# yekaizhou/duet

Measured on AMD Instinct MI355X. Metric: SV support-read marks clustered+phased /sec; bit-exact phased_sv.vcf vs ref, higher is better.
Workload: dtype u32/u64 integer + f64 threshold compares; 1 GPU; BASELINE configs[1]: synthetic 1 contig, 1001116 SV marks / 100000 candidates / 159991 tagged reads, resident in HBM; step = ef_classify + ef_finalize_own, two launches (phasing, E/F; ef_seed_sort 0: ; marks_per_gpu=1001116, candidates_per_gpu=100000, reads_per_gpu=159991, parallelism=contig-sharded x1, svlen_thres=50, suppread_thres=2, device_preheat_steps=2500

## Files before the change

### duet_amd/csrc/duet_ef.hip

```cpp

#include <hip/hip_runtime.h>
#include <hip/hip_ext.h>
#include <stdint.h>
#include <stdio.h>
#include <stdlib.h>
#include <string.h>
#include <string>
#include <vector>

#include "duet_ef.h"
#include "duet_internal.h"

#pragma clang fp contract(off)

namespace {

#ifdef DUET_STAMPS
#define STAMP(k, i) do { if (threadIdx.x == 0 && p.stamps) p.stamps[((size_t)(k) * 65536 + blockIdx.x) * 8 + (i)] = wall_clock64(); } while (0)
#else
#define STAMP(k, i) do { } while (0)
#endif

#include "duet_seeds.hip.h"

constexpr uint32_t kPcMax = DUET_PC_MAX;

constexpr uint8_t kNeedNearest = 4;
constexpr uint8_t kClass2 = 8;
constexpr uint8_t kClass2Slow = 16;
constexpr uint8_t kDivZero = 32;

constexpr int kCandPerBlock = 256;
constexpr int kChunk = 3072;
constexpr int kStageIt = kChunk / (kCandPerBlock * 4);
constexpr int kSmallK = 64;
constexpr int kSortThreads = 1024;
constexpr uint32_t kSortLds = 15360;
constexpr uint32_t kLongCnt = 16;
constexpr uint32_t kLongTiles = 256;
constexpr uint32_t kMaxRuns = 32;
constexpr uint32_t kSeedTab = 4096;
constexpr uint32_t kFewRuns = 4;
constexpr uint32_t kOneLds = 4096;
constexpr uint32_t kC2Quota = 64;
constexpr int kC2Groups = 2;
constexpr int kC2Words = 2 + 6 * kC2Groups;

struct Vote {
    uint32_t hap1, hap2, hap0, allhap;
    uint64_t t1, t2;
};

__device__ int decide(int cls, const Vote &v, uint32_t deg, uint32_t svread, uint32_t refread)
{
    const bool hp_le = deg != 0 && 4ull * v.allhap <= 3ull * deg, hp_gt = deg != 0 && !hp_le;
    const double a1 = v.hap1 > 0 ? (double)v.t1 / (double)v.hap1 : 0.0;
    const double a2 = v.hap2 > 0 ? (double)v.t2 / (double)v.hap2 : 0.0;
    const double sv_ratio = (double)svread / (double)((uint64_t)svread + (uint64_t)refread);
    const uint64_t lo = v.t1 < v.t2 ? v.t1 : v.t2;
    const uint64_t hi = v.t1 < v.t2 ? v.t2 : v.t1;
    const double totsc_ratio = lo > 0 ? (double)hi / (double)lo : 0.0;
    const uint64_t onehap = lo == 0 ? hi : 0;
    const double diff = fabs(a2 - a1);
    int pred = 0;
    if (cls == 0) {
        if (sv_ratio == 1.0 && svread >= 4) pred = 3;
    } else if (cls == 2) {
        if (sv_ratio >= 0.72) {
            if (diff <= 1369.50) { if (svread >= 3) pred = 3; }
            else { if (v.hap0 >= 6) pred = 3; }
        }
    } else {
        const bool gate = (hp_le && diff <= 2400.0) || hp_gt;
        if (onehap != 0) {
            if (sv_ratio <= 0.24) pred = 0;
            else if (sv_ratio <= 0.9) { if (gate) pred = a1 > 0 ? 1 : 2; }
            else { if (gate) pred = 3; }
        } else {
            if (sv_ratio <= 0.3) pred = 0;
            else if (sv_ratio <= 0.45) pred = refread > 10 ? 0 : (v.t1 > v.t2 ? 1 : 2);
            else if (sv_ratio <= 0.75) pred = totsc_ratio <= 9.72 ? 3 : (v.t1 > v.t2 ? 1 : 2);
            else pred = 3;
        }
    }
    return pred;
}

__device__ __forceinline__ int decide01_int(int cls, const Vote &v, uint32_t deg, uint32_t svread, uint32_t refread, bool &need_fp)
{
    const uint64_t sr64 = (uint64_t)svread + (uint64_t)refread;
    const uint32_t sr = (uint32_t)sr64, s = svread;
    const uint32_t t1 = (uint32_t)v.t1, t2 = (uint32_t)v.t2, h1 = v.hap1, h2 = v.hap2;
    need_fp = (sr64 >> 26) != 0 || ((v.t1 | v.t2) >> 21) != 0 || ((h1 | h2) >> 8) != 0 || (deg >> 28) != 0;
    if (cls == 0) return (refread == 0 && svread >= 4) ? 3 : 0;
    const uint32_t s4 = s << 2, s10 = (s << 3) + (s << 1), s20 = s10 << 1, s25 = (s << 4) + (s << 3) + s;
    const uint32_t sr3 = (sr << 1) + sr, sr6 = sr3 << 1, sr9 = (sr << 3) + sr;
    const bool le024 = s25 <= sr6, le09 = s10 <= sr9, le03 = s10 <= sr3, le045 = s20 <= sr9, le075 = s4 <= sr3;
    const bool hp_le = deg != 0 && (v.allhap << 2) <= (deg << 1) + deg, hp_gt = deg != 0 && !hp_le;
    const uint32_t lo = t1 < t2 ? t1 : t2, hi = t1 < t2 ? t2 : t1;
    bool diff_le = true;
    if (h1 != 0 && h2 != 0) {
        const int32_t N = (int32_t)__umul24(t2, h1) - (int32_t)__umul24(t1, h2);
        const uint32_t A = (uint32_t)(N < 0 ? -N : N), B = __umul24(__umul24(h1, h2), 2400u);
        need_fp = need_fp || (A == B && t1 != 0 && t2 != 0);
        diff_le = A <= B;
    } else if ((h1 | h2) != 0) {
        diff_le = (h1 != 0 ? t1 : t2) <= __umul24(h1 | h2, 2400u);
    }
    const bool gate = (hp_le && diff_le) || hp_gt;
    int pred = 0;
    if (lo == 0 && hi != 0) {
        if (le024) pred = 0;
        else if (le09) { if (gate) pred = (h1 != 0 && t1 != 0) ? 1 : 2; }
        else { if (gate) pred = 3; }
    } else {
        const bool ratio_le = lo == 0 || __umul24(hi, 25u) <= __umul24(lo, 243u);
        if (le03) pred = 0;
        else if (le045) pred = refread > 10 ? 0 : (t1 > t2 ? 1 : 2);
        else if (le075) pred = ratio_le ? 3 : (t1 > t2 ? 1 : 2);
        else pred = 3;
    }
    return pred;
}

__device__ __forceinline__ uint32_t find_contig(const uint32_t *__restrict__ ctg_off, uint32_t K, uint32_t c)
{
    uint32_t lo = 0, hi = K;
    while (hi - lo > 1) {
        const uint32_t mid = (lo + hi) >> 1;
        if (ctg_off[mid] <= c) lo = mid; else hi = mid;
    }
    return lo;
}

struct Params {
    uint32_t K, C, M;
    uint32_t n_reads;
    const uint64_t *untagged;
    const uint64_t *read_tag;
    const uint32_t *cand_pos, *cand_svlen, *cand_svread, *cand_refread;
    const uint8_t *cand_gt_ok;
    const uint32_t *cand_off, *mark_read;
    uint32_t svlen_thres, suppread_thres;
    const uint32_t *ctg_off;
    const uint8_t *ctg_start;
    const uint32_t *blk_ctg;
    uint64_t *blk_rec;
    uint64_t *seed_ent;
    uint32_t *onebuf;
    uint32_t one_cap;
    uint32_t *tmpbuf;
    uint32_t *n_one;
    uint32_t *c2rec;
    uint32_t c2_fixed, c2_cap;
    uint32_t *status;
    uint8_t *out_pred;
    uint32_t *out_ps;
    uint32_t n_small;
    uint32_t ctg_small[kSmallK + 1];
    const uint32_t *dyn_c;
    const uint16_t *cand_contig;
    uint32_t dbg;
    uint32_t heavy_t;
    unsigned long long *stamps;
};


struct CandState {
    uint32_t first_ps = kEmpty;
    bool multi = false;
    uint32_t ps_a = kEmpty, ps_b = kEmpty, n_a = 0, n_b = 0, nv = 0;
    uint32_t a1 = 0, a2 = 0, b1 = 0, b2 = 0;
    uint32_t tb1 = 0, tb2 = 0;
    uint64_t TA1 = 0, TA2 = 0;
    bool more = false;

    __device__ __forceinline__ uint32_t n_ps() const { return first_ps == kEmpty ? 0u : (multi ? 2u : 1u); }
    __device__ __forceinline__ uint32_t seed() const { return ps_a; }
};

__device__ __forceinline__ uint32_t sel0(unsigned long long mask, uint32_t v)
{
    uint32_t d;
    asm("v_cndmask_b32_e64 %0, 0, %1, %2" : "=v"(d) : "v"(v), "s"(mask));
    return d;
}
__device__ __forceinline__ uint32_t selv(unsigned long long mask, uint32_t a, uint32_t b)
{
    uint32_t d;
    asm("v_cndmask_b32_e64 %0, %1, %2, %3" : "=v"(d) : "v"(a), "v"(b), "s"(mask));
    return d;
}
__device__ __forceinline__ uint32_t inc(uint32_t x, unsigned long long mask)
{
    uint32_t d;
    asm("v_addc_co_u32_e64 %0, vcc, 0, %1, %2" : "=v"(d) : "v"(x), "s"(mask) : "vcc");
    return d;
}

__device__ __forceinline__ void consume_range(CandState &st, const uint64_t *s_tag, uint32_t lo, uint32_t hi, uint32_t cs)
{
    uint32_t mn = st.first_ps;
    uint32_t mx = st.first_ps == kEmpty ? 0u : st.first_ps + 1u;
    uint32_t pa1 = 0, pa2 = 0, pb1 = 0, pb2 = 0;
    unsigned long long has_a = __ballot(st.ps_a != kEmpty), has_b = __ballot(st.ps_b != kEmpty), more = 0;
    uint32_t nv = 0, nb = 0, ps_a = st.ps_a, ps_b = st.ps_b;
    const uint64_t *q = s_tag + (lo < hi ? lo - cs : 0u), *qe = q + (lo < hi ? hi - lo : 0u);
    for (; q < qe; ++q) {
        const uint64_t tag = *q;
        const uint32_t ps = (uint32_t)tag, w = (uint32_t)(tag >> 32);
        const uint32_t pc = w & 0x3FFFFFFFu;
        const unsigned long long vm = __ballot(pc <= kPcMax);
        const unsigned long long m1 = __ballot((int32_t)w >= 0x40000000), m2 = __ballot((int32_t)w < -0x40000000);
        mn = min(mn, ps);
        mx = max(mx, ps + 1u);
        nv = inc(nv, vm);
        ps_a = selv(vm & ~has_a, ps_a, ps);
        has_a |= vm;
        const unsigned long long ina = vm & __ballot(ps == ps_a), rest = vm ^ ina;
        ps_b = selv(rest & ~has_b, ps_b, ps);
        has_b |= rest;
        const unsigned long long inb = rest & __ballot(ps == ps_b);
        more |= rest ^ inb;
        nb = inc(nb, inb);
        const uint32_t pcx = pc | (1u << 24);
        pa1 += sel0(ina & m1, pcx); pa2 += sel0(ina & m2, pcx);
        pb1 += sel0(inb & m1, pcx); pb2 += sel0(inb & m2, pcx);
    }
    const uint32_t lane = threadIdx.x & 63u;
    st.ps_a = ps_a; st.ps_b = ps_b;
    st.more = st.more || ((more >> lane) & 1ull) != 0ull;
    st.multi = st.multi || (mn != kEmpty && mn + 1u != mx);
    st.first_ps = mn;
    st.nv += nv; st.n_b += nb;
    st.n_a = st.more ? (st.ps_a != kEmpty ? 1u : 0u) : st.nv - st.n_b;
    st.a1 += pa1 >> 24; st.a2 += pa2 >> 24; st.b1 += pb1 >> 24; st.b2 += pb2 >> 24;
    st.TA1 += pa1 & 0xFFFFFFu; st.TA2 += pa2 & 0xFFFFFFu;
    st.tb1 += pb1 & 0xFFFFFFu; st.tb2 += pb2 & 0xFFFFFFu;
}

__device__ __forceinline__ uint32_t wave_sum(uint32_t v)
{
    v += (uint32_t)__builtin_amdgcn_update_dpp(0, (int)v, 0xB1, 0xF, 0xF, false);
    v += (uint32_t)__builtin_amdgcn_update_dpp(0, (int)v, 0x4E, 0xF, 0xF, false);
    v += (uint32_t)__builtin_amdgcn_update_dpp(0, (int)v, 0x124, 0xF, 0xF, false);
    v += (uint32_t)__builtin_amdgcn_update_dpp(0, (int)v, 0x128, 0xF, 0xF, false);
    v += (uint32_t)__builtin_amdgcn_update_dpp(0, (int)v, 0x142, 0xA, 0xF, false);
    v += (uint32_t)__builtin_amdgcn_update_dpp(0, (int)v, 0x143, 0xC, 0xF, false);
    return (uint32_t)__builtin_amdgcn_readlane((int)v, 63);
}

template <uint32_t J>
__device__ __forceinline__ uint32_t lane_xor(uint32_t v)
{
    if constexpr (J == 1) return (uint32_t)__builtin_amdgcn_update_dpp(0, (int)v, 0xB1, 0xF, 0xF, false);
    else if constexpr (J == 2) return (uint32_t)__builtin_amdgcn_update_dpp(0, (int)v, 0x4E, 0xF, 0xF, false);
    else if constexpr (J == 4) {
        const int r = __builtin_amdgcn_update_dpp((int)v, (int)v, 0x104, 0xF, 0x5, false);
        return (uint32_t)__builtin_amdgcn_update_dpp(r, (int)v, 0x114, 0xF, 0xA, false);
    } else if constexpr (J == 8) return (uint32_t)__builtin_amdgcn_update_dpp(0, (int)v, 0x128, 0xF, 0xF, false);
    else return (uint32_t)__shfl_xor((int)v, (int)J, 64);
}

template <uint32_t KK, uint32_t J>
__device__ __forceinline__ uint32_t bitonic_step(uint32_t v, uint32_t lane)
{
    const uint32_t o = lane_xor<J>(v);
    const bool up = KK == 64u || (lane & KK) == 0u, low = (lane & J) == 0u;
    v = (low == up) ? min(v, o) : max(v, o);
    if constexpr (J > 1) return bitonic_step<KK, J / 2>(v, lane);
    else return v;
}
__device__ __forceinline__ uint32_t wave_sort64(uint32_t v, uint32_t lane)
{
    v = bitonic_step<2, 1>(v, lane);
    v = bitonic_step<4, 2>(v, lane);
    v = bitonic_step<8, 4>(v, lane);
    v = bitonic_step<16, 8>(v, lane);
    v = bitonic_step<32, 16>(v, lane);
    return bitonic_step<64, 32>(v, lane);
}

__device__ __forceinline__ void consume_heavy(CandState &st, const uint64_t *s_tag, uint32_t lo, uint32_t hi, uint32_t cs, uint32_t lane,
                                              uint32_t h)
{
    uint32_t first_ps = (uint32_t)__builtin_amdgcn_readlane((int)st.first_ps, h);
    uint32_t ps_a = (uint32_t)__builtin_amdgcn_readlane((int)st.ps_a, h);
    uint32_t ps_b = (uint32_t)__builtin_amdgcn_readlane((int)st.ps_b, h);
    bool multi = false, more = false;
    uint32_t nv = 0, n_a = 0, n_b = 0, a1 = 0, a2 = 0, b1 = 0, b2 = 0;
    uint32_t ta1 = 0, ta2 = 0, tb1 = 0, tb2 = 0;
    for (uint32_t m0 = lo; m0 < hi; m0 += 64u) {
        const uint32_t m = m0 + lane;
        const uint64_t tag = m < hi ? s_tag[m - cs] : kUntagged;
        const uint32_t ps = (uint32_t)tag, w = (uint32_t)(tag >> 32);
        const uint32_t pc = w & 0x3FFFFFFFu, hap = w >> 30;
        const bool voter = pc <= kPcMax;
        const unsigned long long tmask = __ballot(ps != kEmpty);
        if (first_ps == kEmpty && tmask) first_ps = (uint32_t)__builtin_amdgcn_readlane((int)ps, (uint32_t)__ffsll((long long)tmask) - 1u);
        multi = multi || __ballot(ps != first_ps && ps != kEmpty) != 0ull;
        const unsigned long long vmask = __ballot(voter);
        if (ps_a == kEmpty && vmask) ps_a = (uint32_t)__builtin_amdgcn_readlane((int)ps, (uint32_t)__ffsll((long long)vmask) - 1u);
        const bool in_a = voter && ps == ps_a;
        const unsigned long long amask = __ballot(in_a);
        const unsigned long long rmask = vmask & ~amask;
        if (ps_b == kEmpty && rmask) ps_b = (uint32_t)__builtin_amdgcn_readlane((int)ps, (uint32_t)__ffsll((long long)rmask) - 1u);
        const bool in_b = voter && !in_a && ps == ps_b;
        const unsigned long long bmask = __ballot(in_b);
        more = more || (rmask & ~bmask) != 0ull;
        const bool is1 = hap == 1, is2 = hap == 2;
        const unsigned long long m1 = __ballot(is1), m2 = __ballot(is2);
        nv += (uint32_t)__popcll(vmask);
        n_a += (uint32_t)__popcll(amask); n_b += (uint32_t)__popcll(bmask);
        a1 += (uint32_t)__popcll(amask & m1); a2 += (uint32_t)__popcll(amask & m2);
        b1 += (uint32_t)__popcll(bmask & m1); b2 += (uint32_t)__popcll(bmask & m2);
        ta1 += (in_a && is1) ? pc : 0u; ta2 += (in_a && is2) ? pc : 0u;
        tb1 += (in_b && is1) ? pc : 0u; tb2 += (in_b && is2) ? pc : 0u;
    }
    const uint32_t s_a1 = a1 ? wave_sum(ta1) : 0u, s_a2 = a2 ? wave_sum(ta2) : 0u;
    const uint32_t s_b1 = b1 ? wave_sum(tb1) : 0u, s_b2 = b2 ? wave_sum(tb2) : 0u;
    if (lane == h) {
        st.first_ps = first_ps; st.multi = st.multi || multi;
        st.ps_a = ps_a; st.ps_b = ps_b; st.more = st.more || more;
        st.nv += nv; st.n_a += n_a; st.n_b += n_b;
        st.a1 += a1; st.a2 += a2; st.b1 += b1; st.b2 += b2;
        st.TA1 += s_a1; st.TA2 += s_a2; st.tb1 += s_b1; st.tb2 += s_b2;
    }
}

struct TileRecs {
    const ulonglong4 *p;
    __device__ __forceinline__ ulonglong4 operator[](uint32_t b) const { return p[2 * (size_t)b]; }
    __device__ __forceinline__ ulonglong4 second(uint32_t b) const { return p[2 * (size_t)b + 1]; }
};

struct TileShared {
    uint32_t seed[kCandPerBlock];
    uint32_t wcnt[kCandPerBlock / 64], wlast[kCandPerBlock / 64], wclean[kCandPerBlock / 64];
    uint32_t c2n;
    uint32_t c2base;
};

__device__ __forceinline__ void store_summary(const Params &p, uint32_t slot, const CandState &st)
{
    uint32_t *rec = p.c2rec + (size_t)slot * kC2Words;
    const uint32_t ng = (st.n_a != 0) + (st.n_b != 0);
    rec[0] = st.nv; rec[1] = ng;
    rec[2] = st.ps_a; rec[3] = st.n_a; rec[4] = st.a1; rec[5] = st.a2;
    rec[6] = (uint32_t)st.TA1; rec[7] = (uint32_t)st.TA2;
    rec[8] = st.ps_b; rec[9] = st.n_b; rec[10] = st.b1; rec[11] = st.b2; rec[12] = st.tb1; rec[13] = st.tb2;
}

__device__ __forceinline__ uint32_t decide_store(const Params &p, TileShared &sh, uint32_t tile, bool live, uint32_t c,
                                                 bool active, bool divzero, const CandState &st, uint32_t deg,
                                                 uint32_t svread, uint32_t refread, uint32_t &c2_rank)
{
    uint8_t code = 0;
    uint32_t ps_out = 0;
    bool want_seed = false;
    const uint32_t n_ps = st.n_ps();
    const bool c2 = active && n_ps == 2;
    const bool c2_fast = c2 && !st.more && deg < 500000u;
    const uint32_t rank = c2_fast ? atomicAdd(&sh.c2n, 1u) : kEmpty;
    c2_rank = rank;
    if (live) {
        want_seed = (active || divzero) && (n_ps == 1) && st.seed() != kEmpty;
        if (divzero) {
            code = kDivZero;
        } else if (active) {
            if (c2) {
                if (rank < kC2Quota) {
                    const uint32_t slot = tile * kC2Quota + rank;
                    store_summary(p, slot, st);
                    code = kClass2;
                    ps_out = slot;
                } else {
                    code = kClass2Slow;
                }
            } else {
                Vote v;
                v.hap1 = st.a1; v.hap2 = st.a2; v.hap0 = 0;
                v.allhap = st.a1 + st.a2;
                v.t1 = st.TA1; v.t2 = st.TA2;
                bool need_fp = false;
                int pred = (p.dbg & DUET_DBG_EF_FP_DECIDE) ? 0 : decide01_int((int)n_ps, v, deg, svread, refread, need_fp);
                need_fp = need_fp || (p.dbg & DUET_DBG_EF_FP_DECIDE) != 0;
                if (need_fp) pred = decide((int)n_ps, v, deg, svread, refread);
                code = (uint8_t)pred;
                ps_out = st.ps_a == kEmpty ? 0u : st.ps_a;
                if (n_ps == 0 || (st.a1 == 0 && st.a2 == 0)) code |= kNeedNearest;
            }
        }
        p.out_pred[c] = code;
        p.out_ps[c] = ps_out;
    }
    return want_seed ? st.seed() : kEmpty;
}

__device__ __forceinline__ void seeds_tile(const Params &p, TileShared &sh, uint32_t tile, uint32_t tid, uint32_t c,
                                           uint32_t is_start)
{
    const uint32_t seed = sh.seed[tid];
    const bool want_seed = seed != kEmpty;
    const uint32_t lane = tid & 63u, wave = tid >> 6;
    const unsigned long long wmask = __ballot(want_seed);
    const unsigned long long smask = __ballot(is_start != 0);
    const unsigned long long upto = lane == 63 ? ~0ull : ((1ull << (lane + 1)) - 1ull);
    if (lane == 0) {
        if (wmask) {
            const uint32_t li = 63u - (uint32_t)__clzll(wmask);
            sh.wlast[wave] = sh.seed[wave * 64 + li];
            sh.wclean[wave] = (li == 63 || (smask >> (li + 1)) == 0) ? 1u : 0u;
        } else {
            sh.wlast[wave] = kEmpty;
            sh.wclean[wave] = 0;
        }
    }
    __syncthreads();
    bool keep = want_seed;
    if (want_seed) {
        const unsigned long long lower = wmask & (upto >> 1);
        if (lower) {
            const uint32_t pl = 63u - (uint32_t)__clzll(lower);
            const unsigned long long between = smask & upto & ~((1ull << (pl + 1)) - 1ull);
            keep = !(between == 0 && sh.seed[wave * 64 + pl] == seed);
        } else if (wave > 0) {
            keep = !((smask & upto) == 0 && sh.wclean[wave - 1] && sh.wlast[wave - 1] == seed);
        }
    }
    const unsigned long long mask = __ballot(keep);
    if (lane == 0) sh.wcnt[wave] = (uint32_t)__popcll(mask);
    __syncthreads();
    uint32_t before = 0, total = 0;
#pragma unroll
    for (uint32_t w = 0; w < kCandPerBlock / 64; ++w) {
        before += w < wave ? sh.wcnt[w] : 0u;
        total += sh.wcnt[w];
    }
    if (keep) {
        const uint32_t at = before + (uint32_t)__popcll(mask & (upto >> 1));
        const uint64_t e = ((uint64_t)c << 32) | seed;
        if (at < 7) p.blk_rec[(size_t)tile * 8 + 1 + at] = e;
        if (at >= 3) p.seed_ent[(size_t)tile * kCandPerBlock + at] = e;
    }
    if (tid == 0) p.blk_rec[(size_t)tile * 8] = total;
}

__device__ __forceinline__ void stage_load_marks(const Params &p, uint4 (&r)[kStageIt], uint32_t cs, uint32_t m_end, uint32_t tid)
{
#pragma unroll
    for (int it = 0; it < kStageIt; ++it) {
        const uint32_t m = cs + 4u * (tid + it * kCandPerBlock);
        r[it] = *reinterpret_cast<const uint4 *>(p.mark_read + (m < m_end ? m : cs));
    }
}

__device__ __forceinline__ void stage_gather(const Params &p, uint64_t (&t)[4 * kStageIt], const uint4 (&r)[kStageIt])
{
#pragma unroll
    for (int it = 0; it < kStageIt; ++it) {
        const uint32_t idx[4] = {r[it].x, r[it].y, r[it].z, r[it].w};
#pragma unroll
        for (int j = 0; j < 4; ++j) {
            const uint64_t *a = idx[j] < p.n_reads ? p.read_tag + idx[j] : p.untagged;
            t[4 * it + j] = *a;
        }
    }
}

__device__ __forceinline__ void stage_store(uint64_t *s_tag, const uint64_t (&t)[4 * kStageIt], uint32_t cs, uint32_t m_end, uint32_t tid)
{
#pragma unroll
    for (int it = 0; it < kStageIt; ++it) {
        const uint32_t i = 4u * (tid + it * kCandPerBlock);
        if (cs + i < m_end) {
#pragma unroll
            for (int j = 0; j < 4; ++j) s_tag[i + j] = t[4 * it + j];
        }
    }
}

template <bool VEC, bool DYN = false>
__global__ __launch_bounds__(kCandPerBlock, 6) void ef_classify(const Params p)
{
    __shared__ uint64_t s_tag[kChunk];
    __shared__ uint32_t s_off[kCandPerBlock + 1];
    __shared__ TileShared sh;

    const uint32_t tid = threadIdx.x;
    STAMP(0, 0);
    const uint32_t n_cands = DYN ? *p.dyn_c : p.C;
    for (uint32_t tile = blockIdx.x; !DYN || tile * (uint32_t)kCandPerBlock < n_cands; tile += gridDim.x) {
        const uint32_t c0 = tile * kCandPerBlock;
        const uint32_t nc = min((uint32_t)kCandPerBlock, n_cands - c0);
        for (uint32_t i = tid; i <= nc; i += kCandPerBlock) s_off[i] = p.cand_off[c0 + i];
        if (tid == 0) sh.c2n = 0;

        uint32_t svlen = 0, svread = 0, refread = 0, gt_ok = 0, is_start = 0;
        if (tid < nc) {
            svlen = p.cand_svlen[c0 + tid];
            svread = p.cand_svread[c0 + tid];
            refread = p.cand_refread[c0 + tid];
            gt_ok = p.cand_gt_ok[c0 + tid];
            if (DYN) {
                const uint32_t c = c0 + tid;
                if (p.cand_contig) {
                    is_start = (c == 0 || p.cand_contig[c] != p.cand_contig[c - 1]) ? 1u : 0u;
                } else {
                    uint32_t k = p.blk_ctg[tile];
                    while (c >= p.ctg_off[k + 1]) ++k;
                    is_start = c == p.ctg_off[k] ? 1u : 0u;
                }
            } else {
                is_start = p.ctg_start[c0 + tid];
            }
        }
        const bool kept = tid < nc && svlen >= p.svlen_thres && svread >= p.suppread_thres && gt_ok != 0;
        const bool divzero = kept && ((uint64_t)svread + (uint64_t)refread == 0);
        __syncthreads();
        STAMP(0, 1);
        const uint32_t m_begin = s_off[0], m_end = s_off[nc];

        const uint32_t j = tid;
        const bool live = j < nc;
        const bool active = kept && !divzero;
        const uint32_t my_b = live ? s_off[j] : 0, my_e = live ? s_off[j + 1] : 0;
        CandState st;

        const uint32_t base = VEC ? (m_begin & ~3u) : m_begin;
        for (uint32_t cs = base; cs < m_end; cs += kChunk) {
            if (VEC) {
                uint4 r[kStageIt];
                uint64_t t[4 * kStageIt];
                stage_load_marks(p, r, cs, m_end, tid);
                stage_gather(p, t, r);
                stage_store(s_tag, t, cs, m_end, tid);
            } else {
                for (uint32_t i = tid; i < kChunk && cs + i < m_end; i += kCandPerBlock) {
                    const uint32_t r = p.mark_read[cs + i];
                    s_tag[i] = r < p.n_reads ? p.read_tag[r] : kUntagged;
                }
            }
            __syncthreads();
            STAMP(0, 2);
            uint32_t lo = max(my_b, cs);
            const uint32_t hi = min(my_e, cs + (uint32_t)kChunk);
            if (!kept) lo = hi;
            const bool heavy = lo < hi && my_e - my_b > min(p.heavy_t, 255u);
            unsigned long long hm = __ballot(heavy);
            consume_range(st, s_tag, heavy ? hi : lo, hi, cs);
            while (hm) {
                const uint32_t h = (uint32_t)__builtin_amdgcn_readfirstlane((int)((uint32_t)__ffsll((long long)hm) - 1u));
                hm &= hm - 1ull;
                const uint32_t lo_h = (uint32_t)__builtin_amdgcn_readlane((int)lo, h), hi_h = (uint32_t)__builtin_amdgcn_readlane((int)hi, h);
                consume_heavy(st, s_tag, lo_h, hi_h, cs, tid & 63u, h);
            }
            STAMP(0, 3);
            __syncthreads();
        }
        STAMP(0, 4);
        uint32_t c2_rank;
        const uint32_t seed = decide_store(p, sh, tile, live, c0 + j, active, divzero, st, my_e - my_b, svread, refread, c2_rank);
        sh.seed[j] = seed;
        __syncthreads();
        if (sh.c2n > kC2Quota) {
            if (tid == 0) sh.c2base = atomicAdd(&p.status[1], sh.c2n - kC2Quota);
            __syncthreads();
            if (live && c2_rank != kEmpty && c2_rank >= kC2Quota) {
                const uint32_t at = sh.c2base + (c2_rank - kC2Quota);
                if (at < p.c2_cap - p.c2_fixed) {
                    store_summary(p, p.c2_fixed + at, st);
                    p.out_pred[c0 + j] = kClass2;
                    p.out_ps[c0 + j] = p.c2_fixed + at;
                }
            }
        }
        seeds_tile(p, sh, tile, tid, c0 + tid, is_start);
        STAMP(0, 6);
        if (!DYN) break;
        __syncthreads();
    }
}


__device__ void bitonic_sort(uint32_t *a, uint32_t n, uint32_t tid, uint32_t nthreads)
{
    uint32_t lN = 0;
    while ((1u << lN) < n) ++lN;
    const uint32_t pairs = (1u << lN) >> 1;
    for (uint32_t lk = 1; lk <= lN; ++lk) {
        const uint32_t k = 1u << lk, half = k >> 1;
        for (uint32_t i = tid; i < pairs; i += nthreads) {
            const uint32_t base = (i >> (lk - 1)) << lk, off = i & (half - 1);
            const uint32_t x = base + off, y = base + (k - 1 - off);
            if (y < n) {
                const uint32_t ax = a[x], ay = a[y];
                if (ax > ay) { a[x] = ay; a[y] = ax; }
            }
        }
        __syncthreads();
        for (int lj = (int)lk - 2; lj >= 0; --lj) {
            const uint32_t j = 1u << lj;
            for (uint32_t i = tid; i < pairs; i += nthreads) {
                const uint32_t x = ((i >> lj) << (lj + 1)) + (i & (j - 1)), y = x + j;
                if (y < n) {
                    const uint32_t ax = a[x], ay = a[y];
                    if (ax > ay) { a[x] = ay; a[y] = ax; }
                }
            }
            __syncthreads();
        }
    }
}

__device__ bool oddeven_rounds(uint32_t *a, uint32_t n, uint32_t tid, uint32_t nthreads, uint32_t *s_flag, int max_rounds)
{
    for (int r = 0; r < max_rounds; ++r) {
        if (tid == 0) *s_flag = 0;
        __syncthreads();
        for (int par = 0; par < 2; ++par) {
            for (uint32_t i = 2 * tid + par; i + 1 < n; i += 2 * nthreads) {
                const uint32_t x = a[i], y = a[i + 1];
                if (x > y) { a[i] = y; a[i + 1] = x; *s_flag = 1; }
            }
            __syncthreads();
        }
        if (*s_flag == 0) return true;
        __syncthreads();
    }
    return false;
}

__device__ uint32_t block_exscan(uint32_t v, uint32_t tid, uint32_t *s_part , uint32_t nthreads,
                                 uint32_t *total)
{
    const uint32_t lane = tid & 63u, wave = tid >> 6;
    uint32_t x = v;
#pragma unroll
    for (int d = 1; d < 64; d <<= 1) {
        const uint32_t y = __shfl_up(x, d, 64);
        if ((int)lane >= d) x += y;
    }
    if (lane == 63) s_part[wave] = x;
    __syncthreads();
    uint32_t before = 0, tot = 0;
    for (uint32_t w = 0; w < nthreads / 64; ++w) {
        const uint32_t pw = s_part[w];
        before += w < wave ? pw : 0u;
        tot += pw;
    }
    __syncthreads();
    *total = tot;
    return before + x - v;
}

__device__ uint32_t unique_copy(const uint32_t *src, uint32_t n, uint32_t *dst, uint32_t tid, uint32_t nthreads,
                                uint32_t *s_part)
{
    const uint32_t per = (n + nthreads - 1) / nthreads;
    const uint32_t b = min(n, tid * per), e = min(n, b + per);
    uint32_t cnt = 0;
    for (uint32_t i = b; i < e; ++i) cnt += (i == 0 || src[i] != src[i - 1]);
    uint32_t total;
    uint32_t at = block_exscan(cnt, tid, s_part, nthreads, &total);
    for (uint32_t i = b; i < e; ++i)
        if (i == 0 || src[i] != src[i - 1]) dst[at++] = src[i];
    return total;
}

__global__ __launch_bounds__(kSortThreads) void ef_seed_sort(const Params p)
{
    __shared__ __align__(16) uint32_t s_key[kSortLds];
    __shared__ uint32_t s_part[kSortThreads / 64 + 1];
    __shared__ uint32_t s_unsorted;
    __shared__ uint32_t s_nruns, s_run[kMaxRuns + 1];
    __shared__ uint32_t s_nlong, s_long[kLongTiles][2];
    __shared__ uint32_t s_tab[kSeedTab];
    __shared__ uint32_t s_ndist;
    const uint32_t k = blockIdx.x, tid = threadIdx.x;
    STAMP(1, 0);
    const uint32_t c_lo = p.n_small ? p.ctg_small[k] : p.ctg_off[k];
    const uint32_t c_hi = p.n_small ? p.ctg_small[k + 1] : p.ctg_off[k + 1];
    uint32_t *region = p.onebuf + c_lo + k;
    if (c_lo == c_hi) {
        if (tid == 0) { p.n_one[k] = 0; region[0] = 0; }
        return;
    }
    if (tid == 0) { s_unsorted = 0; s_nruns = 0; s_nlong = 0; }
    const uint32_t b_lo = c_lo / kCandPerBlock, b_hi = (c_hi - 1) / kCandPerBlock;
    const uint32_t nb = b_hi - b_lo + 1;
    const uint32_t per = (nb + kSortThreads - 1) / kSortThreads;
    const uint32_t my_lo = min(b_lo + tid * per, b_hi + 1), my_hi = min(my_lo + per, b_hi + 1);
    uint32_t *glist = region + 1;
    auto entry = [&](uint32_t b, uint32_t j, const ulonglong4 &rec) -> uint64_t {
        return j == 0 ? rec.y : (j == 1 ? rec.z : (j == 2 ? rec.w : p.seed_ent[(size_t)b * kCandPerBlock + j]));
    };
    const TileRecs recs{reinterpret_cast<const ulonglong4 *>(p.blk_rec)};
    ulonglong4 rec0 = {0, 0, 0, 0}, recp = {0, 0, 0, 0};
    if (my_lo < my_hi) {
        rec0 = recs[my_lo];
        if (my_lo > b_lo) recp = recs[my_lo - 1];
// ... 519 lines not shown
        const uint32_t c0 = tile * 256u;
        const uint32_t c = c0 + tid;
        const bool live = c < n_cands;
        const uint8_t code = live ? p.out_pred[c] : 0;
        const uint32_t ps_in = live ? p.out_ps[c] : 0;
        if (tid == 0) {
            const uint32_t last = min(c0 + 255u, n_cands - 1);
            const uint32_t k0 = (DYN && p.cand_contig) ? (uint32_t)p.cand_contig[c0] : p.blk_ctg[tile];
            uint32_t k1 = k0;
            while (last >= p.ctg_off[k1 + 1]) ++k1;
            uint32_t any = 0;
            for (uint32_t k = k0; k <= k1; ++k) any |= (p.n_one[k] == 0);
            const uint32_t n0 = p.n_one[k0];
            s_meta[0] = k0;
            s_meta[1] = (k0 == k1 && n0 > 0 && n0 <= kOneLds) ? n0 : kEmpty;
            s_meta[2] = any;
            s_meta[3] = p.ctg_off[k0] + k0 + 1;
        }
        __syncthreads();
        STAMP(2, 1);
        const uint32_t k0 = s_meta[0], n_lds = s_meta[1], any_empty = s_meta[2];
        const bool lds_mode = n_lds != kEmpty;
        if (lds_mode) {
            const uint32_t *src = p.onebuf + s_meta[3];
            for (uint32_t i = tid; i < n_lds; i += 256u) s_one[i] = src[i];
            __syncthreads();
        }
        STAMP(2, 2);
        if (live) finalize_candidate(p, c, code, ps_in, k0, lds_mode, s_one, n_lds, any_empty);
        if (!DYN) break;
        __syncthreads();
    }
}

constexpr uint32_t kOwnMaxTiles = 2048;
constexpr uint32_t kOwnTab = 2048;
constexpr uint32_t kOwnKeys = 1024;

struct OwnArgs {
    TileRecs recs;
    const uint64_t *seed_ent, *read_tag;
    const uint32_t *cand_pos, *cand_off, *cand_svread, *cand_refread, *mark_read, *c2rec;
    uint32_t *out_ps, *status;
    uint8_t *out_pred;
    uint32_t c_lo, c_hi;
};

template <class F>
__device__ __forceinline__ void own_each_entry(TileRecs recs, const uint64_t *seed_ent, uint32_t c_lo, uint32_t c_hi, uint32_t first,
                                               uint32_t stride, F f)
{
    const uint32_t b_lo = c_lo / kCandPerBlock, b_hi = (c_hi - 1) / kCandPerBlock;
    for (uint32_t b = b_lo + first; b <= b_hi; b += stride) {
        const ulonglong4 rec = recs[b];
        const uint32_t cnt = (uint32_t)rec.x;
        for (uint32_t j = 0; j < cnt; ++j) {
            const uint64_t e = j == 0 ? rec.y : (j == 1 ? rec.z : (j == 2 ? rec.w : seed_ent[(size_t)b * kCandPerBlock + j]));
            const uint32_t c = (uint32_t)(e >> 32);
            if (c >= c_lo && c < c_hi) f((uint32_t)e);
        }
    }
}

__device__ __forceinline__ uint32_t own_nearest_walk(const OwnArgs &a, uint32_t pos)
{
    uint32_t best = 0;
    int64_t bd = -1;
    own_each_entry(a.recs, a.seed_ent, a.c_lo, a.c_hi, 0u, 1u, [&](uint32_t ps) {
        const int64_t d = llabs((int64_t)pos - (int64_t)ps);
        if (bd < 0 || d < bd || (d == bd && ps > best)) { bd = d; best = ps; }
    });
    return best;
}
__device__ __forceinline__ bool own_member_walk(const OwnArgs &a, uint32_t key)
{
    bool hit = false;
    own_each_entry(a.recs, a.seed_ent, a.c_lo, a.c_hi, 0u, 1u, [&](uint32_t ps) { hit = hit || ps == key; });
    return hit;
}

template <class F>
__device__ __forceinline__ void own_each_tag(const OwnArgs &a, uint32_t b, uint32_t e, F f)
{
    for (uint32_t m = b; m < e; ++m) {
        const uint32_t r = a.mark_read[m];
        f(r == kEmpty ? kUntagged : a.read_tag[r]);
    }
}

__device__ __forceinline__ void finalize_candidate_walk(const OwnArgs &a, uint32_t c, uint32_t code, uint32_t ps_in)
{
    if (code & kDivZero) {
        atomicOr(&a.status[0], 1u);
        a.out_pred[c] = 0;
        a.out_ps[c] = 0;
        return;
    }
    const uint32_t c_pos = a.cand_pos[c];
    if (code & (kClass2 | kClass2Slow)) {
        Vote v = {0, 0, 0, 0, 0, 0};
        uint32_t ps = 0;
        const uint32_t mb = a.cand_off[c], me = a.cand_off[c + 1];
        if (code & kClass2) {
            const uint32_t *rec = a.c2rec + (size_t)ps_in * kC2Words;
            v.allhap = rec[0];
            const uint32_t ng = rec[1];
            uint32_t best = 0;
            for (uint32_t k = 0; k < (uint32_t)kC2Groups; ++k) {
                const uint32_t *g = rec + 2 + 6 * k;
                if (k < ng && g[1] > best && own_member_walk(a, g[0])) {
                    best = g[1];
                    ps = g[0];
                    v.hap1 = g[2]; v.hap2 = g[3];
                    v.t1 = g[4]; v.t2 = g[5];
                    v.hap0 = v.allhap - v.hap1 - v.hap2;
                }
            }
        } else {
            uint32_t best = 0;
            own_each_tag(a, mb, me, [&](uint64_t t) {
                if (t != kUntagged && tag_pc(t) <= kPcMax) ++v.allhap;
            });
            uint32_t done_ps = kEmpty;
            own_each_tag(a, mb, me, [&](uint64_t t) {
                if (t == kUntagged || tag_pc(t) > kPcMax) return;
                const uint32_t g = tag_ps(t);
                if (g == done_ps || (g == ps && best)) return;
                if (!own_member_walk(a, g)) return;
                uint32_t n = 0, n1 = 0, n2 = 0;
                uint64_t s1 = 0, s2 = 0;
                own_each_tag(a, mb, me, [&](uint64_t u) {
                    if (u == kUntagged || tag_pc(u) > kPcMax || tag_ps(u) != g) return;
                    ++n;
                    const uint32_t hap = tag_hap(u), pc = tag_pc(u);
                    n1 += hap == 1 ? 1u : 0u; s1 += hap == 1 ? pc : 0u;
                    n2 += hap == 2 ? 1u : 0u; s2 += hap == 2 ? pc : 0u;
                });
                done_ps = g;
                if (n > best) {
                    best = n; ps = g;
                    v.hap1 = n1; v.hap2 = n2; v.t1 = s1; v.t2 = s2;
                    v.hap0 = v.allhap - n1 - n2;
                }
            });
        }
        if (v.hap1 == 0 && v.hap2 == 0) ps = own_nearest_walk(a, c_pos);
        a.out_pred[c] = (uint8_t)decide(2, v, me - mb, a.cand_svread[c], a.cand_refread[c]);
        a.out_ps[c] = ps;
        return;
    }
    a.out_pred[c] = (uint8_t)(code & 3u);
    a.out_ps[c] = own_nearest_walk(a, c_pos);
}

__device__ __forceinline__ void lds_barrier() { asm volatile("s_waitcnt lgkmcnt(0)\n\ts_barrier" ::: "memory"); }

__device__ __forceinline__ uint32_t wave_max_u32(uint32_t v)
{
    v = max(v, (uint32_t)__builtin_amdgcn_update_dpp(0, (int)v, 0xB1, 0xF, 0xF, false));
    v = max(v, (uint32_t)__builtin_amdgcn_update_dpp(0, (int)v, 0x4E, 0xF, 0xF, false));
    v = max(v, (uint32_t)__builtin_amdgcn_update_dpp(0, (int)v, 0x124, 0xF, 0xF, false));
    v = max(v, (uint32_t)__builtin_amdgcn_update_dpp(0, (int)v, 0x128, 0xF, 0xF, false));
    v = max(v, (uint32_t)__builtin_amdgcn_update_dpp(0, (int)v, 0x142, 0xA, 0xF, false));
    v = max(v, (uint32_t)__builtin_amdgcn_update_dpp(0, (int)v, 0x143, 0xC, 0xF, false));
    return (uint32_t)__builtin_amdgcn_readlane((int)v, 63);
}

__device__ __forceinline__ void own_sort_set(const uint32_t *s_tab, uint32_t *s_key, uint32_t *s_one, uint32_t *s_part, uint32_t u)
{
    const uint32_t tid = threadIdx.x, lane = tid & 63u, wave = tid >> 6;
    uint32_t mv[kOwnTab / 256u], cnt = 0;
#pragma unroll
    for (uint32_t j = 0; j < kOwnTab / 256u; ++j) {
        mv[j] = s_tab[tid + 256u * j];
        cnt += mv[j] != kEmpty ? 1u : 0u;
    }
    uint32_t x = cnt;
#pragma unroll
    for (int d = 1; d < 64; d <<= 1) {
        const uint32_t y = __shfl_up(x, d, 64);
        if ((int)lane >= d) x += y;
    }
    if (lane == 63) s_part[wave] = x;
    __syncthreads();
    uint32_t at = x - cnt;
#pragma unroll
    for (uint32_t w = 0; w < 4; ++w) at += w < wave ? s_part[w] : 0u;
#pragma unroll
    for (uint32_t j = 0; j < kOwnTab / 256u; ++j)
        if (mv[j] != kEmpty) s_key[at++] = mv[j];
    const uint32_t U = (u + 63u) & ~63u, nblk = U >> 6;
    if (tid < U - u) s_key[u + tid] = kEmpty;
    __syncthreads();
    for (uint32_t b = wave; b < nblk; b += 4u) s_key[b * 64u + lane] = wave_sort64(s_key[b * 64u + lane], lane);
    __syncthreads();
    for (uint32_t i = tid; i < U; i += 256u) {
        const uint32_t me = s_key[i];
        uint32_t rank = 0;
        for (uint32_t b = 0; b < nblk; b += 4u) {
            const uint32_t *b0 = s_key + b * 64u, *b1 = s_key + min(b + 1u, nblk - 1u) * 64u;
            const uint32_t *b2 = s_key + min(b + 2u, nblk - 1u) * 64u, *b3 = s_key + min(b + 3u, nblk - 1u) * 64u;
            uint32_t p0 = 0, p1 = 0, p2 = 0, p3 = 0;
#pragma unroll
            for (uint32_t st = 32; st > 0; st >>= 1) {
                p0 += b0[p0 + st - 1u] < me ? st : 0u;
                p1 += b1[p1 + st - 1u] < me ? st : 0u;
                p2 += b2[p2 + st - 1u] < me ? st : 0u;
                p3 += b3[p3 + st - 1u] < me ? st : 0u;
            }
            p0 += b0[p0] < me ? 1u : 0u;
            p1 += b1[p1] < me ? 1u : 0u;
            p2 += b2[p2] < me ? 1u : 0u;
            p3 += b3[p3] < me ? 1u : 0u;
            rank += p0 + (b + 1u < nblk ? p1 : 0u) + (b + 2u < nblk ? p2 : 0u) + (b + 3u < nblk ? p3 : 0u);
        }
        if (me != kEmpty) s_one[rank] = me;
    }
    __syncthreads();
}

__device__ __forceinline__ void own_vote_from_marks(const uint32_t *mark_read, const uint64_t *read_tag, uint32_t mb, uint32_t me_,
                                                 const uint32_t *s_tab, Vote *vo, uint32_t *pso)
{
    auto each = [&](auto f) {
        for (uint32_t m0 = mb; m0 < me_; m0 += 8) {
            uint32_t r[8];
            uint64_t t[8];
#pragma unroll
            for (int j = 0; j < 8; ++j) r[j] = mark_read[m0 + j < me_ ? m0 + j : mb];
#pragma unroll
            for (int j = 0; j < 8; ++j) t[j] = read_tag[r[j] == kEmpty ? 0u : r[j]];
#pragma unroll
            for (int j = 0; j < 8; ++j)
                if (m0 + j < me_) f(r[j] == kEmpty ? kUntagged : t[j]);
        }
    };
    auto member = [&](uint32_t key) -> bool {
        uint32_t h = (key * 2654435761u) >> (32u - 11u);
        for (;;) {
            const uint32_t v = s_tab[h];
            if (v == key) return true;
            if (v == kEmpty) return false;
            h = (h + 1u) & (kOwnTab - 1u);
        }
    };
    Vote v = {0, 0, 0, 0, 0, 0};
    uint32_t ps = 0, best = 0, done_ps = kEmpty;
    each([&](uint64_t t) {
        if (t != kUntagged && tag_pc(t) <= kPcMax) ++v.allhap;
    });
    each([&](uint64_t t) {
        if (t == kUntagged || tag_pc(t) > kPcMax) return;
        const uint32_t g = tag_ps(t);
        if (g == done_ps || (g == ps && best)) return;
        if (!member(g)) return;
        uint32_t n = 0, n1 = 0, n2 = 0;
        uint64_t s1 = 0, s2 = 0;
        each([&](uint64_t u) {
            if (u == kUntagged || tag_pc(u) > kPcMax || tag_ps(u) != g) return;
            ++n;
            const uint32_t hap = tag_hap(u), pc = tag_pc(u);
            n1 += hap == 1 ? 1u : 0u; s1 += hap == 1 ? pc : 0u;
            n2 += hap == 2 ? 1u : 0u; s2 += hap == 2 ? pc : 0u;
        });
        done_ps = g;
        if (n > best) {
            best = n; ps = g;
            v.hap1 = n1; v.hap2 = n2; v.t1 = s1; v.t2 = s2;
            v.hap0 = v.allhap - n1 - n2;
        }
    });
    *vo = v;
    *pso = ps;
}

__device__ __forceinline__ bool own_probe(uint32_t *s_tab, uint32_t key, uint32_t h)
{
    for (uint32_t probes = 0; probes < kOwnTab; ++probes) {
        const uint32_t old = atomicCAS(&s_tab[h], kEmpty, key);
        if (old == kEmpty) return true;
        if (old == key) return false;
        h = (h + 1u) & (kOwnTab - 1u);
    }
    return false;
}

constexpr uint32_t kOwnWin = 64;

__global__ __launch_bounds__(256) void ef_finalize_own(const Params p)
{
    __shared__ uint32_t s_tab[kOwnTab];
    __shared__ uint32_t s_key[kOwnKeys];
    __shared__ uint32_t s_one[kOwnKeys];
    __shared__ uint32_t s_win[kOwnWin];
    __shared__ uint32_t s_mm[4][2];
    __shared__ uint32_t s_red[4][3];
    __shared__ uint32_t s_part[4];
    __shared__ uint32_t s_nwin;
    __shared__ __align__(8) uint32_t s_c2[kC2Quota * kC2Words];
    const uint32_t tid = threadIdx.x, lane = tid & 63u, wave = tid >> 6;
    STAMP(2, 0);
    if (blockIdx.x == 0 && tid == 0) p.status[1] = 0;
    const uint32_t n_cands = p.C;
    const uint32_t nK = p.n_small;
    auto coff = [&](uint32_t kk) -> uint32_t { return p.ctg_small[kk]; };
    const uint32_t tile = blockIdx.x;
    const uint32_t c0 = tile * 256u, c = c0 + tid;
    const bool live = c < n_cands;
// ... 834 lines not shown
```

Measured before the change: 58.63 billion marks/s.

## Hoist per-tile candidate loads and drop s_off staging in ef_classify

Reorders the Params struct so hot kernel arguments sit together, and pins scalar arguments and pointers into SGPRs with inline asm. Per-tile candidate fields and offsets are issued as early, unconditional, clamped loads before the dyn_c check. This replaces the LDS s_off array and its barrier, reading the block span directly or through a two-word LDS slot. Sched barriers and asm fences are placed around the mark and gather loads so they are issued in batches, and the bounds check in stage_store is removed, so it now writes past m_end into the tile buffer. The aim is lower per-tile latency and fewer barriers, at the cost of extra speculative loads and heavier register pressure.

```diff
diff --git a/duet_amd/csrc/duet_ef.hip b/duet_amd/csrc/duet_ef.hip
--- a/duet_amd/csrc/duet_ef.hip
+++ b/duet_amd/csrc/duet_ef.hip
@@ -136,33 +136,34 @@
 struct Params {
     uint32_t K, C, M;
     uint32_t n_reads;
+    const uint32_t *cand_off, *mark_read;
+    const uint64_t *read_tag;
     const uint64_t *untagged;
-    const uint64_t *read_tag;
-    const uint32_t *cand_pos, *cand_svlen, *cand_svread, *cand_refread;
+    const uint32_t *cand_svlen, *cand_svread, *cand_refread;
     const uint8_t *cand_gt_ok;
-    const uint32_t *cand_off, *mark_read;
+    const uint8_t *ctg_start;
     uint32_t svlen_thres, suppread_thres;
-    const uint32_t *ctg_off;
-    const uint8_t *ctg_start;
-    const uint32_t *blk_ctg;
+    uint32_t heavy_t;
+    uint32_t dbg;
+    uint8_t *out_pred;
+    uint32_t *out_ps;
     uint64_t *blk_rec;
     uint64_t *seed_ent;
+    uint32_t *c2rec;
+    uint32_t *status;
+    uint32_t c2_fixed, c2_cap;
+    unsigned long long *stamps;
+    const uint32_t *dyn_c;
+    const uint16_t *cand_contig;
+    const uint32_t *blk_ctg;
+    const uint32_t *ctg_off;
+    const uint32_t *cand_pos;
     uint32_t *onebuf;
     uint32_t one_cap;
     uint32_t *tmpbuf;
     uint32_t *n_one;
-    uint32_t *c2rec;
-    uint32_t c2_fixed, c2_cap;
-    uint32_t *status;
-    uint8_t *out_pred;
-    uint32_t *out_ps;
     uint32_t n_small;
     uint32_t ctg_small[kSmallK + 1];
-    const uint32_t *dyn_c;
-    const uint16_t *cand_contig;
-    uint32_t dbg;
-    uint32_t heavy_t;
-    unsigned long long *stamps;
 };
 
 
@@ -327,6 +328,8 @@
         st.TA1 += s_a1; st.TA2 += s_a2; st.tb1 += s_b1; st.tb2 += s_b2;
     }
 }
+
+__device__ __forceinline__ void lds_barrier() { asm volatile("s_waitcnt lgkmcnt(0)\n\ts_barrier" ::: "memory"); }
 
 struct TileRecs {
     const ulonglong4 *p;
@@ -446,37 +449,46 @@
     if (tid == 0) p.blk_rec[(size_t)tile * 8] = total;
 }
 
-__device__ __forceinline__ void stage_load_marks(const Params &p, uint4 (&r)[kStageIt], uint32_t cs, uint32_t m_end, uint32_t tid)
+__device__ __forceinline__ void issue_fence()
+{
+    asm volatile("" ::: "memory");
+    __builtin_amdgcn_sched_barrier(0);
+}
+
+__device__ __forceinline__ void stage_load_marks(const uint32_t *__restrict__ mark_read, uint4 (&r)[kStageIt], uint32_t cs, uint32_t m_end,
+                                                 uint32_t tid)
 {
 #pragma unroll
     for (int it = 0; it < kStageIt; ++it) {
         const uint32_t m = cs + 4u * (tid + it * kCandPerBlock);
-        r[it] = *reinterpret_cast<const uint4 *>(p.mark_read + (m < m_end ? m : cs));
-    }
-}
-
-__device__ __forceinline__ void stage_gather(const Params &p, uint64_t (&t)[4 * kStageIt], const uint4 (&r)[kStageIt])
+        r[it] = *reinterpret_cast<const uint4 *>(mark_read + (m < m_end ? m : cs));
+    }
+    issue_fence();
+}
+
+__device__ __forceinline__ void stage_gather(const uint64_t *__restrict__ read_tag, const uint64_t *__restrict__ untagged, uint32_t n_reads,
+                                             uint64_t (&t)[4 * kStageIt], const uint4 (&r)[kStageIt])
 {
 #pragma unroll
     for (int it = 0; it < kStageIt; ++it) {
-        const uint32_t idx[4] = {r[it].x, r[it].y, r[it].z, r[it].w};
+        uint32_t idx[4] = {r[it].x, r[it].y, r[it].z, r[it].w};
+        asm volatile("" : "+v"(idx[0]), "+v"(idx[1]), "+v"(idx[2]), "+v"(idx[3])::"memory");
 #pragma unroll
         for (int j = 0; j < 4; ++j) {
-            const uint64_t *a = idx[j] < p.n_reads ? p.read_tag + idx[j] : p.untagged;
+            const uint64_t *a = idx[j] < n_reads ? read_tag + idx[j] : untagged;
             t[4 * it + j] = *a;
         }
-    }
-}
-
-__device__ __forceinline__ void stage_store(uint64_t *s_tag, const uint64_t (&t)[4 * kStageIt], uint32_t cs, uint32_t m_end, uint32_t tid)
+        issue_fence();
+    }
+}
+
+__device__ __forceinline__ void stage_store(uint64_t *s_tag, const uint64_t (&t)[4 * kStageIt], uint32_t tid)
 {
 #pragma unroll
     for (int it = 0; it < kStageIt; ++it) {
         const uint32_t i = 4u * (tid + it * kCandPerBlock);
-        if (cs + i < m_end) {
-#pragma unroll
-            for (int j = 0; j < 4; ++j) s_tag[i + j] = t[4 * it + j];
-        }
+#pragma unroll
+        for (int j = 0; j < 4; ++j) s_tag[i + j] = t[4 * it + j];
     }
 }
 
@@ -484,47 +496,81 @@
 __global__ __launch_bounds__(kCandPerBlock, 6) void ef_classify(const Params p)
 {
     __shared__ uint64_t s_tag[kChunk];
-    __shared__ uint32_t s_off[kCandPerBlock + 1];
+    __shared__ uint32_t s_span[2];
     __shared__ TileShared sh;
 
     const uint32_t tid = threadIdx.x;
     STAMP(0, 0);
-    const uint32_t n_cands = DYN ? *p.dyn_c : p.C;
-    for (uint32_t tile = blockIdx.x; !DYN || tile * (uint32_t)kCandPerBlock < n_cands; tile += gridDim.x) {
-        const uint32_t c0 = tile * kCandPerBlock;
+    const uint32_t C = p.C, n_reads = p.n_reads, svlen_thres = p.svlen_thres, suppread_thres = p.suppread_thres;
+    const uint32_t heavy_t = min(p.heavy_t, 255u);
+    const uint32_t *__restrict__ const cand_off = p.cand_off, *__restrict__ const mark_read = p.mark_read;
+    const uint64_t *__restrict__ const read_tag = p.read_tag, *__restrict__ const untagged = p.untagged;
+    const uint32_t *__restrict__ const cand_svlen = p.cand_svlen, *__restrict__ const cand_svread = p.cand_svread;
+    const uint32_t *__restrict__ const cand_refread = p.cand_refread;
+    const uint8_t *__restrict__ const cand_gt_ok = p.cand_gt_ok, *__restrict__ const ctg_start = p.ctg_start;
+    asm volatile("" ::"s"(C), "s"(n_reads), "s"(svlen_thres), "s"(suppread_thres), "s"(heavy_t), "s"(cand_off), "s"(mark_read),
+                 "s"(read_tag), "s"(untagged), "s"(cand_svlen), "s"(cand_svread), "s"(cand_refread), "s"(cand_gt_ok), "s"(ctg_start));
+    asm volatile("" ::"s"(p.dbg), "s"(p.out_pred), "s"(p.out_ps), "s"(p.blk_rec), "s"(p.seed_ent), "s"(p.c2rec), "s"(p.status),
+                 "s"(p.c2_fixed), "s"(p.c2_cap));
+    uint32_t n_cands = C;
+    for (uint32_t tile = blockIdx.x;; tile += gridDim.x) {
+        const uint32_t c0 = tile * kCandPerBlock, c = c0 + tid;
+        const uint32_t ic = min(c, C - 1u);
+        const uint32_t o0_ld = cand_off[min(c, C)], o1_ld = cand_off[min(c + 1u, C)];
+        const uint32_t svlen_ld = cand_svlen[ic], svread_ld = cand_svread[ic], refread_ld = cand_refread[ic], gt_ld = cand_gt_ok[ic];
+        uint32_t start_ld = 0, cc0_ld = 0, cc1_ld = 0, mb_ld = 0, me_ld = 0;
+        if constexpr (DYN) {
+            if (p.cand_contig) {
+                cc0_ld = p.cand_contig[ic];
+                cc1_ld = p.cand_contig[max(ic, 1u) - 1u];
+            }
+        } else {
+            start_ld = ctg_start[ic];
+            mb_ld = cand_off[c0];
+            me_ld = cand_off[min(c0 + (uint32_t)kCandPerBlock, C)];
+        }
+        if constexpr (DYN) {
+            uint32_t zero = 0;
+            asm volatile("" : "+s"(zero));
+            n_cands = p.dyn_c[zero];
+            if (c0 >= n_cands) break;
+        }
         const uint32_t nc = min((uint32_t)kCandPerBlock, n_cands - c0);
-        for (uint32_t i = tid; i <= nc; i += kCandPerBlock) s_off[i] = p.cand_off[c0 + i];
+        asm volatile("" ::"v"(o0_ld), "v"(o1_ld), "v"(svlen_ld), "v"(svread_ld), "v"(refread_ld), "v"(gt_ld), "v"(start_ld), "v"(cc0_ld),
+                     "v"(cc1_ld));
         if (tid == 0) sh.c2n = 0;
-
-        uint32_t svlen = 0, svread = 0, refread = 0, gt_ok = 0, is_start = 0;
-        if (tid < nc) {
-            svlen = p.cand_svlen[c0 + tid];
-            svread = p.cand_svread[c0 + tid];
-            refread = p.cand_refread[c0 + tid];
-            gt_ok = p.cand_gt_ok[c0 + tid];
-            if (DYN) {
-                const uint32_t c = c0 + tid;
-                if (p.cand_contig) {
-                    is_start = (c == 0 || p.cand_contig[c] != p.cand_contig[c - 1]) ? 1u : 0u;
-                } else {
-                    uint32_t k = p.blk_ctg[tile];
-                    while (c >= p.ctg_off[k + 1]) ++k;
-                    is_start = c == p.ctg_off[k] ? 1u : 0u;
-                }
-            } else {
-                is_start = p.ctg_start[c0 + tid];
-            }
-        }
-        const bool kept = tid < nc && svlen >= p.svlen_thres && svread >= p.suppread_thres && gt_ok != 0;
+        const bool live = tid < nc;
+        const uint32_t svlen = svlen_ld, svread = svread_ld, refread = refread_ld, gt_ok = gt_ld;
+        uint32_t is_start = 0;
+        if constexpr (DYN) {
+            if (p.cand_contig) {
+                is_start = (live && (c == 0 || cc0_ld != cc1_ld)) ? 1u : 0u;
+            } else if (live) {
+                uint32_t k = p.blk_ctg[tile];
+                while (c >= p.ctg_off[k + 1]) ++k;
+                is_start = c == p.ctg_off[k] ? 1u : 0u;
+            }
+        } else {
+            is_start = live ? start_ld : 0u;
+        }
+        const bool kept = live && svlen >= svlen_thres && svread >= suppread_thres && gt_ok != 0;
         const bool divzero = kept && ((uint64_t)svread + (uint64_t)refread == 0);
-        __syncthreads();
+        uint32_t m_begin, m_end;
+        if constexpr (DYN) {
+            if (tid == 0) s_span[0] = o0_ld;
+            if (tid == nc - 1u) s_span[1] = o1_ld;
+            lds_barrier();
+            m_begin = s_span[0]; m_end = s_span[1];
+        } else {
+            m_begin = mb_ld; m_end = me_ld;
+        }
+        m_begin = (uint32_t)__builtin_amdgcn_readfirstlane((int)m_begin);
+        m_end = (uint32_t)__builtin_amdgcn_readfirstlane((int)m_end);
         STAMP(0, 1);
-        const uint32_t m_begin = s_off[0], m_end = s_off[nc];
 
         const uint32_t j = tid;
-        const bool live = j < nc;
         const bool active = kept && !divzero;
-        const uint32_t my_b = live ? s_off[j] : 0, my_e = live ? s_off[j + 1] : 0;
+        const uint32_t my_b = live ? o0_ld : 0, my_e = live ? o1_ld : 0;
         CandState st;
 
         const uint32_t base = VEC ? (m_begin & ~3u) : m_begin;
@@ -532,13 +578,13 @@
             if (VEC) {
                 uint4 r[kStageIt];
                 uint64_t t[4 * kStageIt];
-                stage_load_marks(p, r, cs, m_end, tid);
-                stage_gather(p, t, r);
-                stage_store(s_tag, t, cs, m_end, tid);
+                stage_load_marks(mark_read, r, cs, m_end, tid);
+                stage_gather(read_tag, untagged, n_reads, t, r);
+                stage_store(s_tag, t, tid);
             } else {
                 for (uint32_t i = tid; i < kChunk && cs + i < m_end; i += kCandPerBlock) {
-                    const uint32_t r = p.mark_read[cs + i];
-                    s_tag[i] = r < p.n_reads ? p.read_tag[r] : kUntagged;
+                    const uint32_t r = mark_read[cs + i];
+                    s_tag[i] = r < n_reads ? read_tag[r] : kUntagged;
                 }
             }
             __syncthreads();
@@ -546,7 +592,7 @@
             uint32_t lo = max(my_b, cs);
             const uint32_t hi = min(my_e, cs + (uint32_t)kChunk);
             if (!kept) lo = hi;
-            const bool heavy = lo < hi && my_e - my_b > min(p.heavy_t, 255u);
+            const bool heavy = lo < hi && my_e - my_b > heavy_t;
             unsigned long long hm = __ballot(heavy);
             consume_range(st, s_tag, heavy ? hi : lo, hi, cs);
             while (hm) {
@@ -1372,8 +1418,6 @@
     a.out_pred[c] = (uint8_t)(code & 3u);
     a.out_ps[c] = own_nearest_walk(a, c_pos);
 }
-
-__device__ __forceinline__ void lds_barrier() { asm volatile("s_waitcnt lgkmcnt(0)\n\ts_barrier" ::: "memory"); }
 
 __device__ __forceinline__ uint32_t wave_max_u32(uint32_t v)
 {
```

Measured after the change: 62.05 billion marks/s (median of 6 runs). 1.06x the previous value.
